# Karthik-Ragunath/RAD-NeRF

Measured on AMD Instinct MI355X. Metric: rendered frames/sec @512x512, higher is better.
Workload: dtype f32; 1 GPU; config[1]: inference 512x512, L=16 hash grid T=2^19 F=2 (xyz; ambient/torso grids tiled T=2^16 as shipped), max 16 steps/ray, 25 FPS pose stream, torso pass on; grid=hash19, engine=fused, frames_per_gpu=2122, table_dtype=f32, audio_batch=8, frames_in_flight=1, loop_launch=split, parallelism=frame-parallel x1

## Files before the change

include/radnerf_fused.h:

```cpp
#ifndef RADNERF_FUSED_H
#define RADNERF_FUSED_H

#include "radnerf_hip.h"

#ifdef __cplusplus
extern "C" {
#endif

typedef struct {
    const void *embeddings;
    const int32_t *offsets;
    uint32_t D, L, H;
    float S;
    uint32_t gridtype;
    int dtype;
} rn_grid_t;

typedef struct {
    const float *amb_w0, *amb_w1, *amb_w2;
    const float *sig_w0, *sig_w1, *sig_w2;
    const float *col_w0, *col_w1;
    uint32_t audio_dim, has_eye, ind_dim;
} rn_nerf_weights_t;

// ... 24 lines not shown
    float min_near;
    const uint8_t *bitfield;
    float bound, dt_gamma;
    uint32_t max_steps, cascade, grid_size;
    float T_thresh;
    float *nears, *fars;
    float *weights_sum, *depth, *image;
    int32_t *rays_alive_a, *rays_alive_b;
    float *rays_t;
    float *xyzs, *dirs, *deltas;
    float *sigmas, *rgbs;
    int32_t *state;
    uint32_t *block_counts;
    int32_t *live_slots;
    uint32_t order_w;
} rn_head_t;

int rn_head_begin(const rn_head_t *h, rn_stream_t stream);
int rn_head_iterate(const rn_head_t *h, const rn_grid_t *grid_xyz, const rn_grid_t *grid_amb, const float *packed,
                    const float *bias, uint32_t first_iter, uint32_t n_iters, int mlp_dtype, rn_stream_t stream);
#define RN_LOOP_FIRST_MARCHED 1u
#define RN_LOOP_CLOSE_FRAME 2u
#define RN_LOOP_COOP 4u
int rn_head_iterate_ex(const rn_head_t *h, const rn_grid_t *grid_xyz, const rn_grid_t *grid_amb, const float *packed,
                       const float *bias, uint32_t first_iter, uint32_t n_iters, int mlp_dtype, uint32_t flags,
                       rn_stream_t stream);
int rn_frame_begin(const rn_head_t *h, const float *pose, float fx, float fy, float cx, float cy, uint32_t W,
                   rn_stream_t stream);
int rn_head_reschedule(const rn_head_t *h, uint32_t iter_done, uint32_t schedule_N, const int32_t *alive_total,
                       rn_stream_t stream);
// ... 24 lines not shown
                         float thresh, const float *poses6, const float *ind_code, float torso_shrink,
                         const rn_torso_weights_t *w, const float *packed, const rn_grid_t *grid_torso, const float *bg_in,
                         float *bg_out, float *torso_alpha, float *image, const float *weights_sum, float *depth,
                         const float *nears, const float *fars, uint8_t *image_u8, rn_stream_t stream);

int rn_torso_mask(const float *bg_coords, uint32_t N, const float *density_grid_torso, uint32_t grid_size, float thresh,
                  uint8_t *mask, rn_stream_t stream);

int rn_blend_frame(float *image, const float *weights_sum, const float *bg, float *depth, const float *nears,
                   const float *fars, uint32_t N, uint8_t *image_u8, rn_stream_t stream);

size_t rn_occupancy_workspace(uint32_t C, uint32_t H);
int rn_occupancy_points(uint32_t C, uint32_t H, float bound, const float *noise, uint32_t seed, float *xyzs, rn_stream_t stream);
int rn_occupancy_update(const float *sigmas, float density_scale, float *density_grid, uint32_t C, uint32_t H, float decay,
                        float density_thresh, uint8_t *bitfield, float *stats, void *workspace, rn_stream_t stream);
int rn_mark_untrained_grid(const float *poses, uint32_t n_poses, uint32_t pose_stride, double fx, double fy, double cx, double cy,
                           uint32_t C, uint32_t H, float bound, float *density_grid, rn_stream_t stream);
int rn_torso_grid_points(uint32_t H, const float *noise, uint32_t seed, float *xys, rn_stream_t stream);
int rn_torso_grid_update(const float *alphas, float *density_grid_torso, uint32_t H, float decay, float *stats, rn_stream_t stream);
uint32_t rn_hash_u01_bits(uint32_t seed, uint32_t idx);

typedef struct {
    const float *conv_w[4], *conv_b[4];
    const float *fc_w[2], *fc_b[2];
    const float *att_conv_w[5], *att_conv_b[5];
    const float *att_fc_w, *att_fc_b;
    uint32_t dim_in, dim_aud, has_att;
} rn_audio_weights_t;
#define RN_AUDIO_SEQ 8
#define RN_AUDIO_WIN 16
// ... 66 lines not shown
```

rad-nerf_amd/csrc/rn_dda_dev.h:

```cpp
#pragma once

#include "rn_common.h"

namespace rn {

constexpr float kSqrt3 = 1.7320508075688772f;


__device__ __forceinline__ int mip_from_pos(float x, float y, float z, float max_cascade) {
    const float mx = fmaxf(fabsf(x), fmaxf(fabsf(y), fabsf(z)));
    int e;
    frexpf(mx, &e);
    return (int)fminf(max_cascade - 1, fmaxf(0.0f, (float)e));
}
__device__ __forceinline__ int mip_from_dt(float dt, float H, float max_cascade) {
    const float mx = (float)((double)(dt * H) * 0.5);
    int e;
    frexpf(mx, &e);
    return (int)fminf(max_cascade - 1, fmaxf(0.0f, (float)e));
}

struct Dda {
    float ox, oy, oz, dx, dy, dz, rdx, rdy, rdz;
    float rH, H3, bound, dt_gamma, dt_min, dt_max, far, Cf, Hf;
// ... 103 lines not shown

    __device__ __forceinline__ void emit(float t, float *xyz, float *dir, float *delta) const {
        EmitSamples{xyz, dir, delta}(*this, 0u, t, clampf(ox + t * dx, -bound, bound), clampf(oy + t * dy, -bound, bound),
                                     clampf(oz + t * dz, -bound, bound), clampf(t * dt_gamma, dt_min, dt_max));
    }

    __device__ __forceinline__ float start(float t, float u) const { return t + clampf(t * dt_gamma, dt_min, dt_max) * u; }

    __device__ __forceinline__ uint32_t march_slot(float t, uint32_t n_step, uint32_t base, float *xyzs, float *dirs, float *deltas) const {
        const uint32_t emitted = walk(t, n_step, EmitSamples{xyzs + (size_t)base * 3, dirs + (size_t)base * 3, deltas + (size_t)base * 2});
        for (uint32_t k = emitted; k < n_step; k++) { deltas[((size_t)base + k) * 2] = 0.0f; deltas[((size_t)base + k) * 2 + 1] = 0.0f; }
        return emitted;
    }
};

}
```

rad-nerf_amd/csrc/rn_head_loop.hip:

```cpp
#include "rn_fused_dev.h"
#include "rn_ray_dev.h"

namespace rn {

constexpr int kLoopBlock = 256;

__device__ __forceinline__ uint32_t policy_n_step(uint32_t N, uint32_t n_alive) {
    uint32_t n_step = n_alive ? N / n_alive : 1u;
    n_step = n_step > 8u ? 8u : n_step;
    return n_step < 1u ? 1u : n_step;
}

__device__ __forceinline__ void next_state(int32_t *st, uint32_t N, uint32_t n_alive, uint32_t step, uint32_t max_steps) {
    const uint32_t n_step = policy_n_step(N, n_alive);
    const bool active = step < max_steps && n_alive > 0;
    st[0] = (int32_t)n_alive;
    st[1] = (int32_t)step;
    st[2] = (int32_t)n_step;
    st[3] = active ? (int32_t)(n_alive * n_step) : 0;
    st[4] = active ? 1 : 0;
    st[5] = 0;
}

__device__ __forceinline__ uint32_t list_live_slots(uint32_t emitted, uint32_t base, int32_t *live_count,
// ... 22 lines not shown
        state[6] = 0;
        for (int i = 8; i < 16; i++) state[i] = 0;
        state[RN_HEAD_ST_HIST] = (int32_t)N;
    }
    if (n >= N) return;
    float near, far;
    begin_ray(n, rays_o + (size_t)n * 3, rays_d + (size_t)n * 3, aabb, min_near, nears, fars, rays_t, weights_sum, depth, image, near, far);
    rays_alive[n] = (int32_t)alive_order(n, order_w);
}

__global__ void __launch_bounds__(kLoopBlock)
k_head_march(const int32_t *__restrict__ st, const int32_t *__restrict__ rays_alive, const float *__restrict__ rays_t,
             const float *__restrict__ rays_o, const float *__restrict__ rays_d, float bound, float dt_gamma,
             uint32_t max_steps, uint32_t C, uint32_t H, const uint8_t *__restrict__ grid,
             const float *__restrict__ fars, float *__restrict__ xyzs, float *__restrict__ dirs, float *__restrict__ deltas, int32_t *__restrict__ stats,
             uint32_t *__restrict__ block_live, int32_t *__restrict__ live_count, int32_t *__restrict__ live_slots) {
    if (!st[4]) return;
    const uint32_t n_alive = (uint32_t)st[0], n_step = (uint32_t)st[2];
    const uint32_t n = blockIdx.x * kLoopBlock + threadIdx.x;
    uint32_t emitted = 0;
    const uint32_t base = n * n_step;
    if (n < n_alive) {
        const int index = rays_alive[n];
        Dda s;
        s.init(rays_o + (size_t)index * 3, rays_d + (size_t)index * 3, bound, dt_gamma, max_steps, C, H, grid, fars[index]);
        emitted = s.march_slot(rays_t[index], n_step, base, xyzs, dirs, deltas);
    }
    __shared__ uint32_t sh[kLoopBlock / kWave + 1];
    const uint32_t total = list_live_slots(emitted, base, live_count, live_slots, sh);
    if (threadIdx.x == 0) block_live[blockIdx.x] = total;
    if (n == 0) { atomicAdd(&stats[RN_HEAD_ST_ITERS], 1); atomicAdd(&stats[RN_HEAD_ST_SLOTS], (int32_t)(n_alive * n_step)); }
}

struct RaySource {
    const float *pose;
    float fx, fy, cx, cy;
    uint32_t W;
};

__global__ void __launch_bounds__(kLoopBlock)
k_frame_begin(RaySource rs, float *__restrict__ rays_o, float *__restrict__ rays_d, const float *__restrict__ aabb, uint32_t N,
              float min_near, uint32_t max_steps, float bound, float dt_gamma, uint32_t C, uint32_t H,
              const uint8_t *__restrict__ grid, float *__restrict__ nears, float *__restrict__ fars, float *__restrict__ weights_sum,
              float *__restrict__ depth, float *__restrict__ image, int32_t *__restrict__ rays_alive, float *__restrict__ rays_t,
              int32_t *__restrict__ state, uint32_t order_w, float *__restrict__ xyzs, float *__restrict__ dirs,
              float *__restrict__ deltas, uint32_t *__restrict__ block_live, int32_t *__restrict__ live_slots) {
    const uint32_t n = blockIdx.x * kLoopBlock + threadIdx.x;
    if (n == 0) {
        next_state(state, N, N, 0, max_steps);
        for (int i = 8; i < 16; i++) state[i] = 0;
        state[RN_HEAD_ST_HIST] = (int32_t)N;
        atomicAdd(&state[RN_HEAD_ST_ITERS], 1);
        atomicAdd(&state[RN_HEAD_ST_SLOTS], (int32_t)N);
    }
    uint32_t emitted = 0;
    if (n < N) {
        const uint32_t ray = alive_order(n, order_w);
        float o[3], d[3];
        if (rs.pose) {
            pinhole_ray(ray, rs.W, rs.fx, rs.fy, rs.cx, rs.cy, rs.pose, o, d);
#pragma unroll
            for (int k = 0; k < 3; k++) { rays_d[(size_t)ray * 3 + k] = d[k]; rays_o[(size_t)ray * 3 + k] = o[k]; }
        } else {
#pragma unroll
            for (int k = 0; k < 3; k++) { o[k] = rays_o[(size_t)ray * 3 + k]; d[k] = rays_d[(size_t)ray * 3 + k]; }
        }
        float near, far;
        begin_ray(ray, o, d, aabb, min_near, nears, fars, rays_t, weights_sum, depth, image, near, far);
        rays_alive[n] = (int32_t)ray;
        Dda s;
        s.init(o, d, bound, dt_gamma, max_steps, C, H, grid, far);
        emitted = s.march_slot(near, 1u, n, xyzs, dirs, deltas);
    }
    __shared__ uint32_t sh[kLoopBlock / kWave + 1];
    const uint32_t total = list_live_slots(emitted, n, state + 6, live_slots, sh);
    if (threadIdx.x == 0) block_live[blockIdx.x] = total;
}

constexpr uint32_t kTagShift = 10;
constexpr uint32_t kTagMask = (1u << 22) - 1u;
constexpr uint32_t kBarrierPolls = 1u << 20;

template <bool COOP>
__device__ __forceinline__ void composite_chunk(uint32_t c, uint32_t n_alive, uint32_t n_step, float T_thresh,
                                                int32_t *__restrict__ rays_alive, float *__restrict__ rays_t,
                                                const float *__restrict__ sigmas, const float *__restrict__ rgbs,
// ... 30 lines not shown
    if (blockIdx.x == 0 && threadIdx.x == 0) st_next[6] = 0;
    const uint32_t n_alive = (uint32_t)st[0], n_step = (uint32_t)st[2];
    if (blockIdx.x * kLoopBlock >= n_alive) return;
    composite_chunk<false>(blockIdx.x, n_alive, n_step, T_thresh, rays_alive, rays_t, sigmas, rgbs, deltas, weights_sum, depth, image,
                           block_counts, wave_cnt);
}

struct MarchArgs {
    const float *rays_t, *rays_o, *rays_d, *fars;
    float bound, dt_gamma;
    uint32_t cascade, grid_size;
    const uint8_t *grid;
    float *xyzs, *dirs, *deltas;
    uint32_t *block_live_next;
    int32_t *live_slots;
};

__device__ __forceinline__ void loop_idle(const int32_t *__restrict__ st, int32_t *__restrict__ st_next, int32_t *__restrict__ stats,
                                          uint32_t close_frame, uint32_t iter) {
    if (blockIdx.x == 0 && threadIdx.x < 8) st_next[threadIdx.x] = st[threadIdx.x];
    if (close_frame && blockIdx.x == 0 && threadIdx.x == 0) { stats[6] = 0; stats[8 + 6] = 0; }
    if (blockIdx.x == 0 && threadIdx.x == 0 && iter + 1 < 32) stats[RN_HEAD_ST_HIST + iter + 1] = 0;
}

template <bool MARCH, bool COOP>
__device__ __forceinline__ void compact_chunk(uint32_t c, uint32_t n_blocks, const int32_t *__restrict__ st, int32_t *__restrict__ st_next,
                                              uint32_t N, uint32_t max_steps, const int32_t *__restrict__ rays_in,
                                              int32_t *__restrict__ rays_out, const uint32_t *__restrict__ block_counts,
                                              const uint32_t *__restrict__ block_live, int32_t *__restrict__ stats, const MarchArgs &m,
                                              uint32_t close_frame, uint32_t iter, uint32_t tag = 0) {
// ... 60 lines not shown
        if (close_frame) {
            if (active_next) atomicAdd(&stats[RN_HEAD_ST_UNFINISHED], 1);
            stats[6] = 0; stats[8 + 6] = 0;
        }
        if (MARCH && active_next) {
            st_next[5] = (int32_t)n_blocks;
            atomicAdd(&stats[RN_HEAD_ST_ITERS], 1);
            atomicAdd(&stats[RN_HEAD_ST_SLOTS], (int32_t)(n_next * n_step_next));
        }
    }
    if constexpr (MARCH) {
        if (!active_next) return;
        uint32_t emitted = 0;
        const uint32_t base = slot * n_step_next;
        if (keep) {
            Dda s;
            s.init(m.rays_o + (size_t)v * 3, m.rays_d + (size_t)v * 3, m.bound, m.dt_gamma, max_steps, m.cascade, m.grid_size, m.grid,
                   m.fars[v]);
            emitted = s.march_slot(m.rays_t[v], n_step_next, base, m.xyzs, m.dirs, m.deltas);
        }
        __shared__ uint32_t sh[kLoopBlock / kWave + 1];
        const uint32_t total = list_live_slots(emitted, base, st_next + 6, m.live_slots, sh);
        if (threadIdx.x == 0) m.block_live_next[c] = total;
    }
}

template <bool MARCH>
__global__ void __launch_bounds__(kLoopBlock)
k_head_compact(const int32_t *__restrict__ st, int32_t *__restrict__ st_next, uint32_t N, uint32_t max_steps,
               const int32_t *__restrict__ rays_in, int32_t *__restrict__ rays_out,
               const uint32_t *__restrict__ block_counts, const uint32_t *__restrict__ block_live, int32_t *__restrict__ stats,
               MarchArgs m, uint32_t close_frame, uint32_t iter) {
    if (!st[4]) { loop_idle(st, st_next, stats, close_frame, iter); return; }
// ... 82 lines not shown
               "head_iterate: mlp_dtype must be RN_F32, RN_F16 or RN_F32_SPLIT");
    RN_REQUIRE(packed && bias && ((uintptr_t)packed & 15u) == 0, "head_iterate: packed/bias");
    if (int rc = check_fused_grid(grid_xyz, 3, "head_iterate(xyz grid)")) return rc;
    if (int rc = check_fused_grid(grid_amb, 2, "head_iterate(ambient grid)")) return rc;
    hipStream_t s = as_stream(stream);
    const dim3 rgrid(div_up(h->N, kLoopBlock)), rblock(kLoopBlock);
    const uint32_t nb = div_up(h->N, kLoopBlock) + 1;
    uint32_t *block_live[2] = {h->block_counts + nb, h->block_counts + 2 * nb};
    for (uint32_t it = first_iter; it < first_iter + n_iters; it++) {
        int32_t *st = h->state + (it & 1u) * 8, *st_next = h->state + ((it + 1) & 1u) * 8;
        int32_t *alive = (it & 1u) ? h->rays_alive_b : h->rays_alive_a;
        int32_t *alive_next = (it & 1u) ? h->rays_alive_a : h->rays_alive_b;
        if (it == first_iter && !(flags & RN_LOOP_FIRST_MARCHED))
            hipLaunchKernelGGL(k_head_march, rgrid, rblock, 0, s, st, alive, h->rays_t, h->rays_o, h->rays_d, h->bound,
                               h->dt_gamma, h->max_steps, h->cascade, h->grid_size, h->bitfield, h->fars, h->xyzs, h->dirs,
                               h->deltas, h->state, block_live[it & 1u], st + 6, h->live_slots);
        run_fused(h->xyzs, h->dirs, h->deltas, h->N, h->live_slots ? st + 6 : st + 3, grid_xyz, grid_amb, packed, bias, h->bound,
                  h->sigmas, h->rgbs, nullptr, mlp_dtype, s, h->live_slots);
        const MarchArgs m{h->rays_t, h->rays_o, h->rays_d, h->fars, h->bound, h->dt_gamma, h->cascade, h->grid_size, h->bitfield,
                          h->xyzs, h->dirs, h->deltas, block_live[(it + 1) & 1u], h->live_slots};
        const bool march_next = it + 1 < first_iter + n_iters;
        const uint32_t close = (!march_next && (flags & RN_LOOP_CLOSE_FRAME)) ? 1u : 0u;
        if (flags & RN_LOOP_COOP) {
            const dim3 cgrid(rgrid.x < kStepGrid ? rgrid.x : kStepGrid);
            uint32_t a_N = h->N, a_max = h->max_steps, a_close = march_next ? 0u : close, a_it = it;
            float a_T = h->T_thresh;
            const int32_t *a_st = st;
            int32_t *a_st_next = st_next, *a_alive = alive, *a_alive_next = alive_next, *a_state = h->state;
            float *a_rays_t = h->rays_t, *a_ws = h->weights_sum, *a_depth = h->depth, *a_image = h->image;
            const float *a_sig = h->sigmas, *a_rgb = h->rgbs, *a_deltas = h->deltas;
            uint32_t *a_counts = h->block_counts;
            const uint32_t *a_live = block_live[it & 1u];
            MarchArgs a_m = m;
            void *args[] = {&a_st, &a_st_next, &a_N, &a_max, &a_T, &a_alive, &a_alive_next, &a_rays_t, &a_sig, &a_rgb, &a_deltas, &a_ws,
                            &a_depth, &a_image, &a_counts, &a_live, &a_state, &a_m, &a_close, &a_it};
// ... 21 lines not shown

int rn_head_iterate(const rn_head_t *h, const rn_grid_t *grid_xyz, const rn_grid_t *grid_amb, const float *packed,
                    const float *bias, uint32_t first_iter, uint32_t n_iters, int mlp_dtype, rn_stream_t stream) {
    return rn_head_iterate_ex(h, grid_xyz, grid_amb, packed, bias, first_iter, n_iters, mlp_dtype, 0u, stream);
}

int rn_frame_begin(const rn_head_t *h, const float *pose, float fx, float fy, float cx, float cy, uint32_t W, rn_stream_t stream) {
    if (int rc = check_head(h)) return rc;
    RN_REQUIRE(!pose || (fx != 0.0f && fy != 0.0f && W >= 1 && h->N % W == 0), "frame_begin: bad intrinsics / image width");
    const uint32_t order_w = usable_order_w(h->order_w, h->N);
    const uint32_t nb = div_up(h->N, kLoopBlock) + 1;
    const RaySource rs{pose, fx, fy, cx, cy, W ? W : 1u};
    hipLaunchKernelGGL(k_frame_begin, dim3(div_up(h->N, kLoopBlock)), dim3(kLoopBlock), 0, as_stream(stream), rs,
                       const_cast<float *>(h->rays_o), const_cast<float *>(h->rays_d), h->aabb, h->N, h->min_near, h->max_steps, h->bound,
                       h->dt_gamma, h->cascade, h->grid_size, h->bitfield, h->nears, h->fars, h->weights_sum, h->depth, h->image,
                       h->rays_alive_a, h->rays_t, h->state, order_w, h->xyzs, h->dirs, h->deltas, h->block_counts + nb, h->live_slots);
    return check_launch("frame_begin");
}

int rn_head_check_done(const rn_head_t *h, uint32_t iters_done, rn_stream_t stream) {
    if (int rc = check_head(h)) return rc;
    hipLaunchKernelGGL(k_head_check_done, dim3(1), dim3(64), 0, as_stream(stream), h->state + (iters_done & 1u) * 8,
                       h->state + RN_HEAD_ST_UNFINISHED);
    return check_launch("head_check_done");
}

int rn_head_reschedule(const rn_head_t *h, uint32_t iter_done, uint32_t schedule_N, const int32_t *alive_total,
                       rn_stream_t stream) {
    if (int rc = check_head(h)) return rc;
    RN_REQUIRE(alive_total && schedule_N >= h->N, "head_reschedule: alive_total is null or schedule_N < N");
    hipLaunchKernelGGL(k_head_reschedule, dim3(1), dim3(64), 0, as_stream(stream), h->state + ((iter_done + 1) & 1u) * 8,
// ... 6 lines not shown
```

rad-nerf_amd/csrc/rn_occupancy.hip:

```cpp
#include "rn_common.h"

#include "../../include/radnerf_fused.h"

#include <math.h>

namespace rn {

constexpr int kOccBlock = 256;

struct CascadeConsts {
    float scale[16];
    float half[16];
};

__global__ void __launch_bounds__(kOccBlock)
k_occ_points(uint32_t C, uint32_t H, CascadeConsts cc, const float *__restrict__ noise, uint32_t seed, float *__restrict__ xyzs) {
    const uint32_t H3 = H * H * H;
    const uint32_t i = blockIdx.x * kOccBlock + threadIdx.x;
    if (i >= C * H3) return;
    const uint32_t cas = i / H3, mo = i - cas * H3;
    const uint32_t c[3] = {morton3D_invert(mo), morton3D_invert(mo >> 1), morton3D_invert(mo >> 2)};
    const float hm1 = (float)(H - 1);
#pragma unroll
    for (int d = 0; d < 3; d++) {
// ... 51 lines not shown
    const uint32_t n = blockIdx.x * kOccBlock + threadIdx.x;
    if (n >= N) return;
    const float thresh = stats[1];
    const float4 a = reinterpret_cast<const float4 *>(grid)[(size_t)n * 2];
    const float4 b = reinterpret_cast<const float4 *>(grid)[(size_t)n * 2 + 1];
    uint32_t bits = 0;
    bits |= (a.x > thresh) ? 1u : 0u;
    bits |= (a.y > thresh) ? 2u : 0u;
    bits |= (a.z > thresh) ? 4u : 0u;
    bits |= (a.w > thresh) ? 8u : 0u;
    bits |= (b.x > thresh) ? 16u : 0u;
    bits |= (b.y > thresh) ? 32u : 0u;
    bits |= (b.z > thresh) ? 64u : 0u;
    bits |= (b.w > thresh) ? 128u : 0u;
    bitfield[n] = (uint8_t)bits;
}

constexpr int kPoseChunk = 64;

__global__ void __launch_bounds__(kOccBlock)
k_mark_untrained(const float *__restrict__ poses, uint32_t n_poses, uint32_t pose_stride, float cx_fx, float cy_fy, uint32_t C,
                 uint32_t H, CascadeConsts cc, float *__restrict__ grid) {
    __shared__ float sp[kPoseChunk][12];
    const uint32_t H3 = H * H * H, total = C * H3;
    const uint32_t i = blockIdx.x * kOccBlock + threadIdx.x;
    const bool in_range = i < total;
    const uint32_t cas = in_range ? i / H3 : 0u, mo = i - cas * H3;
    float w[3] = {0.0f, 0.0f, 0.0f};
    float margin = 0.0f;
    if (in_range) {
// ... 98 lines not shown

int rn_occupancy_update(const float *sigmas, float density_scale, float *density_grid, uint32_t C, uint32_t H, float decay,
                        float density_thresh, uint8_t *bitfield, float *stats, void *workspace, rn_stream_t stream) {
    RN_REQUIRE(sigmas && density_grid && bitfield && stats && workspace, "occupancy_update: null pointer");
    RN_REQUIRE(C >= 1 && C <= 16 && H >= 2 && H <= 1024 && (H * H * H) % 8 == 0, "occupancy_update: bad C / H");
    RN_REQUIRE(((uintptr_t)density_grid & 15u) == 0 && ((uintptr_t)workspace & 7u) == 0, "occupancy_update: alignment");
    const uint32_t total = C * H * H * H, blocks = div_up(total, kOccBlock);
    double *partial = static_cast<double *>(workspace);
    hipStream_t s = as_stream(stream);
    hipLaunchKernelGGL(k_occ_update, dim3(blocks), dim3(kOccBlock), 0, s, sigmas, density_scale, density_grid, C, H, decay, partial);
    hipLaunchKernelGGL(k_occ_mean, dim3(1), dim3(kOccBlock), 0, s, partial, blocks, total, density_thresh, stats);
    hipLaunchKernelGGL(k_occ_pack, dim3(div_up(total / 8, kOccBlock)), dim3(kOccBlock), 0, s, density_grid, total / 8, stats, bitfield);
    return check_launch("occupancy_update");
}

int rn_mark_untrained_grid(const float *poses, uint32_t n_poses, uint32_t pose_stride, double fx, double fy, double cx, double cy,
                           uint32_t C, uint32_t H, float bound, float *density_grid, rn_stream_t stream) {
    RN_REQUIRE(poses && density_grid && n_poses >= 1 && pose_stride >= 12, "mark_untrained_grid: bad arguments");
    RN_REQUIRE(C >= 1 && C <= 16 && H >= 2 && H <= 1024, "mark_untrained_grid: bad C / H");
    const uint32_t total = C * H * H * H;
    hipLaunchKernelGGL(k_mark_untrained, dim3(div_up(total, kOccBlock)), dim3(kOccBlock), 0, as_stream(stream), poses, n_poses,
                       pose_stride, (float)(cx / fx), (float)(cy / fy), C, H,
                       cascade_consts(C, H, (double)bound), density_grid);
    return check_launch("mark_untrained_grid");
}

int rn_torso_grid_points(uint32_t H, const float *noise, uint32_t seed, float *xys, rn_stream_t stream) {
    RN_REQUIRE(xys && H >= 2 && H <= 1024, "torso_grid_points: bad arguments");
    const double half = 1.0 / (double)H;
    hipLaunchKernelGGL(k_torso_points, dim3(div_up(H * H, kOccBlock)), dim3(kOccBlock), 0, as_stream(stream), H, (float)(1.0 - half),
// ... 21 lines not shown
```

rad-nerf_amd/radnerf/fused.py:

```python
import ctypes as C

import numpy as np
import os

import torch

import radnerf_hip as hip
from radnerf_hip.abi import (RN_F16, RN_F32, RN_F32_SPLIT, RN_HEAD_ST_HIST, RN_HEAD_ST_ITERS, RN_HEAD_ST_SLOTS, RN_HEAD_ST_STALLED,
                             RN_HEAD_ST_UNFINISHED, RN_HEAD_STATE_INTS, RN_LOOP_CLOSE_FRAME, RN_LOOP_COOP, RN_LOOP_FIRST_MARCHED,
                             GridT, HeadT, NerfWeightsT, TorsoWeightsT)

_lib = hip._lib


def _grid_desc(enc, table):
    g = GridT()
    g.embeddings, g.offsets = table.data_ptr(), enc.offsets.data_ptr()
    g.D, g.L, g.H = enc.input_dim, enc.num_levels, enc.base_resolution
    g.S = float(np.log2(enc.per_level_scale))
    g.gridtype = enc.gridtype_id
    g.dtype = RN_F16 if table.dtype == torch.float16 else RN_F32
    return g


# ... 46 lines not shown

    def __init__(self, model):
        if not supported(model):
            raise RuntimeError("fused engine: unsupported network shape; use engine='ops'")
        self.model = model
        self.dev = model.density_bitfield.device
        n_packed = max(int(_lib.rn_nerf_packed_floats()), int(_lib.rn_nerf_packed_floats_h16()),
                       int(_lib.rn_nerf_packed_floats_split()))
        self.packed = torch.empty(n_packed, dtype=torch.float32, device=self.dev)
        self.mlp_dtype = RN_F32
        self.loop_hint = None
        self.bias = torch.empty(int(_lib.rn_nerf_bias_floats()), dtype=torch.float32, device=self.dev)
        self.tpacked = (torch.empty(int(_lib.rn_torso_packed_floats()), dtype=torch.float32, device=self.dev)
                        if model.torso else None)
        self._versions = None
        self._N = 0
        self._zero_eye = torch.zeros(1, dtype=torch.float32, device=self.dev)

    def _weights(self):
        m = self.model
        ws = head_weights(m)
        if m.torso:
            ws += torso_weights(m)
        return ws

    def refresh(self):
        ws = self._weights()
        tables = [self.model.encoder.embeddings, self.model.encoder_ambient.embeddings]
        if self.model.torso:
            tables.append(self.model.torso_encoder.embeddings)
        mlp = {"f32": RN_F32, "f16": RN_F16, "f32x2": RN_F32_SPLIT}[
            getattr(getattr(self.model, "opt", None), "mlp_dtype", "f32")]
        half = bool(getattr(getattr(self.model, "opt", None), "half_tables", False))
        versions = tuple((w._version, w.data_ptr()) for w in ws + tables) + (mlp, half)
        if versions == self._versions:
            return
        m = self.model
        for w in ws:
            if w.dtype != torch.float32 or not w.is_contiguous():
                raise RuntimeError("fused engine: MLP weights must be contiguous float32")
        self.nw = weights_desc(ws[:8], m.audio_dim, int(m.exp_eye), m.individual_dim)
# ... 4 lines not shown
                  RN_F32_SPLIT: "rn_nerf_pack_weights_split"}[mlp]
        hip.call(packer, C.byref(self.nw), hip.ptr(self.packed), hip.stream())
        if m.torso:
            self.tw = torso_weights_desc(ws[8:14], m.individual_dim_torso)
            hip.call("rn_torso_pack_weights", C.byref(self.tw), hip.ptr(self.tpacked), hip.stream())
        if half:
            encs = [m.encoder, m.encoder_ambient] + ([m.torso_encoder] if m.torso else [])
            self.tables = [hip.aligned(e.half_table()) for e in encs]
        else:
            self.tables = [hip.aligned(t.detach()) for t in tables]
        self.gx = _grid_desc(m.encoder, self.tables[0])
        self.gw = _grid_desc(m.encoder_ambient, self.tables[1])
        self.gt = _grid_desc(m.torso_encoder, self.tables[2]) if m.torso else None
        self._versions = versions

    def scratch(self, N):
        if N == self._N:
            return
        d, f32, i32 = self.dev, torch.float32, torch.int32
        self.nears = torch.empty(N, dtype=f32, device=d)
        self.fars = torch.empty(N, dtype=f32, device=d)
        self.rays_alive = torch.empty(2, N, dtype=i32, device=d)
        self.rays_t = torch.empty(N, dtype=f32, device=d)
        self.samples = torch.empty(N * 8, dtype=f32, device=d)
        self.sigmas = torch.empty(N, dtype=f32, device=d)
        self.rgbs = torch.empty(N, 3, dtype=f32, device=d)
        self.state = torch.zeros(RN_HEAD_STATE_INTS, dtype=i32, device=d)
        self.stats_prev = [0, 0, 0]
        self.block_counts = torch.zeros(3 * ((N + 255) // 256 + 1), dtype=i32, device=d)
        self.live_slots = torch.empty(N, dtype=i32, device=d)
# ... 202 lines not shown
    h = HeadT()
    h.rays_o, h.rays_d, h.N = rays_o.data_ptr(), rays_d.data_ptr(), N
    h.aabb, h.min_near = model.aabb_infer.data_ptr(), float(model.min_near)
    h.bitfield, h.bound, h.dt_gamma = model.density_bitfield.data_ptr(), float(model.bound), float(dt_gamma)
    h.max_steps, h.cascade, h.grid_size, h.T_thresh = int(max_steps), int(model.cascade), int(model.grid_size), float(T_thresh)
    h.nears, h.fars = st.nears.data_ptr(), st.fars.data_ptr()
    h.weights_sum, h.depth, h.image = weights_sum.data_ptr(), depth.data_ptr(), image.data_ptr()
    h.rays_alive_a, h.rays_alive_b = st.rays_alive[0].data_ptr(), st.rays_alive[1].data_ptr()
    h.rays_t = st.rays_t.data_ptr()
    h.xyzs = st.samples.data_ptr()
    h.dirs = st.samples.data_ptr() + N * 3 * 4
    h.deltas = st.samples.data_ptr() + N * 6 * 4
    h.sigmas, h.rgbs = st.sigmas.data_ptr(), st.rgbs.data_ptr()
    h.state, h.block_counts = st.state.data_ptr(), st.block_counts.data_ptr()
    h.live_slots = st.live_slots.data_ptr() if (getattr(model.opt, "live_list", True) and os.environ.get("RN_LIVE_LIST", "1") != "0") else None
    h.order_w = int(getattr(model, "ray_order_width", 0) or 0)

    shard = getattr(model, "shard_schedule", None)
    merged = shard is None and getattr(model.opt, "frame_kernels", "merged") == "merged"
    n_iters = int(max_steps) if st.loop_hint is None else min(int(max_steps), st.loop_hint)
    if merged:
        if ray_source is not None:
            pose, (fx, fy, cx, cy), W = ray_source
            pose = pose.reshape(-1, 4)[:4].contiguous().float()
            hip.call("rn_frame_begin", C.byref(h), hip.ptr(pose), float(fx), float(fy), float(cx), float(cy), int(W), s)
        else:
            hip.call("rn_frame_begin", C.byref(h), None, 0.0, 0.0, 0.0, 0.0, 0, s)
        hip.call("rn_head_iterate_ex", C.byref(h), C.byref(st.gx), C.byref(st.gw), hip.ptr(st.packed), hip.ptr(bias), 0, n_iters,
                 st.mlp_dtype, RN_LOOP_FIRST_MARCHED | RN_LOOP_CLOSE_FRAME | loop_flags(model), s)
    else:
# ... 80 lines not shown
```

rad-nerf_amd/radnerf/occupancy.py:

```python
import random

import torch

import radnerf_hip as hip

_lib = hip._lib


class _Scratch:

    def __init__(self, model):
        dev = model.density_bitfield.device
        n = model.cascade * model.grid_size ** 3
        self.xyzs = torch.empty(n, 3, dtype=torch.float32, device=dev)
        self.sigmas = torch.empty(n, dtype=torch.float32, device=dev)
        self.stats = torch.zeros(2, dtype=torch.float32, device=dev)
        self.ws = torch.zeros(int(_lib.rn_occupancy_workspace(model.cascade, model.grid_size)), dtype=torch.uint8, device=dev)
        if model.torso:
            g2 = model.grid_size ** 2
            self.xys = torch.empty(g2, 2, dtype=torch.float32, device=dev)
            self.alphas = torch.empty(g2, 1, dtype=torch.float32, device=dev)
            self.bg = torch.empty(g2, 3, dtype=torch.float32, device=dev)
            self.stats_torso = torch.zeros(1, dtype=torch.float32, device=dev)

# ... 13 lines not shown
    if noise.numel() != n * dims:
        raise ValueError(f"jitter noise must hold {n} x {dims} numbers")
    return noise, 0


def _density_into(model, xyzs, sigmas, enc_a, eye):
    from . import fused
    if getattr(model.opt, "grid_refresh_engine", "fused") == "fused" and fused.supported(model):
        fused.density_forward(model, xyzs, enc_a, eye, out=sigmas)
        return
    step = 1 << 19
    for lo in range(0, xyzs.shape[0], step):
        sigmas[lo:lo + step] = model.density(xyzs[lo:lo + step], enc_a, eye)["sigma"].reshape(-1).float()


@torch.no_grad()
def refresh_head(model, enc_a, eye, decay=0.95, noise=None):
    sc = _scratch(model)
    Cc, H = int(model.cascade), int(model.grid_size)
    nz, seed = _jitter(noise, Cc * H ** 3, 3, sc.xyzs.device)
    s = hip.stream()
    hip.call("rn_occupancy_points", Cc, H, float(model.bound), hip.ptr(nz), seed, hip.ptr(sc.xyzs), s)
    _density_into(model, sc.xyzs, sc.sigmas, enc_a, eye)
    grid = model.density_grid
    if not grid.is_contiguous():
        raise RuntimeError("density_grid must be contiguous")
    hip.call("rn_occupancy_update", hip.ptr(sc.sigmas), float(model.density_scale), hip.ptr(grid), Cc, H, float(decay),
             float(model.density_thresh), hip.ptr(model.density_bitfield), hip.ptr(sc.stats), hip.ptr(sc.ws), s)
    return sc.stats


@torch.no_grad()
def refresh_torso(model, enc_a, pose6, ind_code, decay=0.95, noise=None):
    from . import fused
    sc = _scratch(model)
    H = int(model.grid_size)
    nz, seed = _jitter(noise, H * H, 2, sc.xys.device)
    s = hip.stream()
    hip.call("rn_torso_grid_points", H, hip.ptr(nz), seed, hip.ptr(sc.xys), s)
    if fused.supported(model):
        fused.torso_forward(model, sc.xys, pose6, ind_code, thresh=-1.0, bg_out=sc.bg, alpha_out=sc.alphas)
    else:
        sc.alphas.copy_(model.forward_torso(sc.xys, pose6, enc_a, ind_code)[0].float())
# ... 24 lines not shown
```

rad-nerf_amd/radnerf_hip/abi.py:

```python
import ctypes as C

_int, _u32, _f32, _f64, _sz, _ptr, _P = C.c_int, C.c_uint32, C.c_float, C.c_double, C.c_size_t, C.c_void_p, C.POINTER

RN_F32, RN_F16 = 0, 1
RN_LAYOUT_LBC, RN_LAYOUT_BLC, RN_LAYOUT_BLC_LEVELMAJOR = 0, 1, 2

RN_F32_SPLIT = 2
RN_HEAD_STATE_INTS = 64
RN_LOOP_FIRST_MARCHED, RN_LOOP_CLOSE_FRAME, RN_LOOP_COOP = 1, 2, 4
RN_HEAD_ST_ACTIVE, RN_HEAD_ST_ITERS, RN_HEAD_ST_LIVE, RN_HEAD_ST_SLOTS = 4, 16, 17, 18
RN_HEAD_ST_UNFINISHED, RN_HEAD_ST_STALLED, RN_HEAD_ST_HIST = 19, 22, 32


class GridT(C.Structure):
    c_name = "rn_grid_t"
    _fields_ = [("embeddings", _ptr), ("offsets", _ptr), ("D", _u32), ("L", _u32), ("H", _u32), ("S", _f32),
                ("gridtype", _u32), ("dtype", _int)]


class NerfWeightsT(C.Structure):
    c_name = "rn_nerf_weights_t"
    _fields_ = [("amb_w0", _ptr), ("amb_w1", _ptr), ("amb_w2", _ptr), ("sig_w0", _ptr), ("sig_w1", _ptr),
                ("sig_w2", _ptr), ("col_w0", _ptr), ("col_w1", _ptr), ("audio_dim", _u32), ("has_eye", _u32),
                ("ind_dim", _u32)]


class HeadT(C.Structure):
    c_name = "rn_head_t"
    _fields_ = [("rays_o", _ptr), ("rays_d", _ptr), ("N", _u32), ("aabb", _ptr), ("min_near", _f32),
                ("bitfield", _ptr), ("bound", _f32), ("dt_gamma", _f32), ("max_steps", _u32), ("cascade", _u32),
                ("grid_size", _u32), ("T_thresh", _f32), ("nears", _ptr), ("fars", _ptr), ("weights_sum", _ptr),
                ("depth", _ptr), ("image", _ptr), ("rays_alive_a", _ptr), ("rays_alive_b", _ptr), ("rays_t", _ptr),
                ("xyzs", _ptr), ("dirs", _ptr), ("deltas", _ptr), ("sigmas", _ptr), ("rgbs", _ptr), ("state", _ptr),
                ("block_counts", _ptr), ("live_slots", _ptr), ("order_w", _u32)]


class TorsoWeightsT(C.Structure):
    c_name = "rn_torso_weights_t"
    _fields_ = [("def_w0", _ptr), ("def_w1", _ptr), ("def_w2", _ptr), ("tor_w0", _ptr), ("tor_w1", _ptr),
                ("tor_w2", _ptr), ("ind_dim", _u32)]


class AudioWeightsT(C.Structure):
    c_name = "rn_audio_weights_t"
    _fields_ = [("conv_w", _ptr * 4), ("conv_b", _ptr * 4), ("fc_w", _ptr * 2), ("fc_b", _ptr * 2),
                ("att_conv_w", _ptr * 5), ("att_conv_b", _ptr * 5), ("att_fc_w", _ptr), ("att_fc_b", _ptr),
                ("dim_in", _u32), ("dim_aud", _u32), ("has_att", _u32)]


# ... 92 lines not shown
    "rn_head_iterate_ex": (_int, [_P(HeadT), _P(GridT), _P(GridT), _ptr, _ptr, _u32, _u32, _int, _u32, _ptr]),
    "rn_frame_begin": (_int, [_P(HeadT), _ptr, _f32, _f32, _f32, _f32, _u32, _ptr]),
    "rn_head_reschedule": (_int, [_P(HeadT), _u32, _u32, _ptr, _ptr]),
    "rn_head_check_done": (_int, [_P(HeadT), _u32, _ptr]),
    "rn_torso_packed_floats": (_sz, []),
    "rn_torso_pack_weights": (_int, [_P(TorsoWeightsT), _ptr, _ptr]),
    "rn_torso_fused": (_int, [_ptr, _u32, _ptr, _u32, _f32, _ptr, _ptr, _f32, _P(TorsoWeightsT), _ptr, _P(GridT), _ptr, _ptr,
                              _ptr, _ptr, _ptr]),
    "rn_torso_blend_frame": (_int, [_ptr, _u32, _ptr, _u32, _f32, _ptr, _ptr, _f32, _P(TorsoWeightsT), _ptr, _P(GridT), _ptr,
                                    _ptr, _ptr, _ptr, _ptr, _ptr, _ptr, _ptr, _ptr, _ptr]),
    "rn_torso_mask": (_int, [_ptr, _u32, _ptr, _u32, _f32, _ptr, _ptr]),
    "rn_blend_frame": (_int, [_ptr, _ptr, _ptr, _ptr, _ptr, _ptr, _u32, _ptr, _ptr]),
    "rn_occupancy_workspace": (_sz, [_u32, _u32]),
    "rn_occupancy_points": (_int, [_u32, _u32, _f32, _ptr, _u32, _ptr, _ptr]),
    "rn_occupancy_update": (_int, [_ptr, _f32, _ptr, _u32, _u32, _f32, _f32, _ptr, _ptr, _ptr, _ptr]),
    "rn_mark_untrained_grid": (_int, [_ptr, _u32, _u32, _f64, _f64, _f64, _f64, _u32, _u32, _f32, _ptr, _ptr]),
    "rn_torso_grid_points": (_int, [_u32, _ptr, _u32, _ptr, _ptr]),
    "rn_torso_grid_update": (_int, [_ptr, _ptr, _u32, _f32, _ptr, _ptr]),
    "rn_hash_u01_bits": (_u32, [_u32, _u32]),
    "rn_audio_encode_windows": (_int, [_P(AudioWeightsT), _ptr, _u32, _ptr, _ptr, _ptr]),
    "rn_audio_encode_windows_backward": (_int, [_P(AudioWeightsT), _ptr, _u32, _ptr, _ptr, _P(AudioGradsT), _ptr, _ptr]),
    "rn_audio_train_acts_floats": (_sz, [_u32, _int]),
    "rn_audio_encode_windows_train": (_int, [_P(AudioWeightsT), _ptr, _u32, _ptr, _ptr, _ptr, _ptr]),
    "rn_audio_encode_windows_backward_acts": (_int, [_P(AudioWeightsT), _ptr, _u32, _ptr, _ptr, _P(AudioGradsT), _ptr, _ptr,
                                                     _ptr]),
    "rn_audio_encode_stream": (_int, [_P(AudioWeightsT), _ptr, _u32, _u32, _u32, _ptr, _ptr, _ptr]),
    "rn_audio_smooth": (_int, [_ptr, _u32, _u32, _f32, _ptr, _int, _ptr]),
    "rn_audio_smooth_seq": (_int, [_ptr, _u32, _u32, _f32, _ptr, _int, _ptr, _ptr]),
    "rn_get_rays": (_int, [_ptr, _f32, _f32, _f32, _f32, _u32, _u32, _ptr, _ptr, _ptr]),
    "rn_get_bg_coords": (_int, [_u32, _u32, _ptr, _ptr]),
# ... 60 lines not shown
```

Baseline: 1275 frames/s.

## Clip ray marching to the occupied bounding box of the density bitfield

Adds a kernel that reduces the occupancy bitfield to an integer bounding box of occupied cells. The march kernels then clip each ray's far distance to that box and, for single-cascade grids, skip the start forward to the box entry. This aims to cut the empty-space DDA steps and the ray iterations spent outside occupied geometry. It adds a small bounds-refresh kernel whenever the bitfield changes, plus a host sync in refresh. There is some risk of edge mismatches near the box boundaries.

Result: no change. 1287 frames/s, median of 6 (+0.9%).

```diff
diff --git a/include/radnerf_fused.h b/include/radnerf_fused.h
--- a/include/radnerf_fused.h
+++ b/include/radnerf_fused.h
@@ -62,6 +62,7 @@
     uint32_t *block_counts;
     int32_t *live_slots;
     uint32_t order_w;
+    const int32_t *occ_bounds;
 } rn_head_t;
 
 int rn_head_begin(const rn_head_t *h, rn_stream_t stream);
@@ -116,6 +117,7 @@
 int rn_occupancy_points(uint32_t C, uint32_t H, float bound, const float *noise, uint32_t seed, float *xyzs, rn_stream_t stream);
 int rn_occupancy_update(const float *sigmas, float density_scale, float *density_grid, uint32_t C, uint32_t H, float decay,
                         float density_thresh, uint8_t *bitfield, float *stats, void *workspace, rn_stream_t stream);
+int rn_occupancy_bounds(const uint8_t *bitfield, uint32_t C, uint32_t H, int32_t *bounds, rn_stream_t stream);
 int rn_mark_untrained_grid(const float *poses, uint32_t n_poses, uint32_t pose_stride, double fx, double fy, double cx, double cy,
                            uint32_t C, uint32_t H, float bound, float *density_grid, rn_stream_t stream);
 int rn_torso_grid_points(uint32_t H, const float *noise, uint32_t seed, float *xys, rn_stream_t stream);
diff --git a/rad-nerf_amd/csrc/rn_dda_dev.h b/rad-nerf_amd/csrc/rn_dda_dev.h
--- a/rad-nerf_amd/csrc/rn_dda_dev.h
+++ b/rad-nerf_amd/csrc/rn_dda_dev.h
@@ -1,6 +1,7 @@
 #pragma once
 
 #include "rn_common.h"
+#include "rn_occ_clip_dev.h"
 
 namespace rn {
 
@@ -141,4 +142,21 @@
     }
 };
 
+struct DdaClip : Dda {
+    float t_in;
+
+    __device__ __forceinline__ void set_clip(const int32_t *__restrict__ bounds) {
+        const float o[3] = {ox, oy, oz}, rd[3] = {rdx, rdy, rdz};
+        occ_clip_set(bounds, Hf, mb1, o, rd, dt_max, one_step_skips, far, t_in);
+    }
+
+    __device__ __forceinline__ uint32_t march_slot(float t, uint32_t n_step, uint32_t base, float *xyzs, float *dirs, float *deltas) const {
+        if (!occ_clip_advance(t, t_in, far, dt_max)) {
+            for (uint32_t k = 0; k < n_step; k++) { deltas[((size_t)base + k) * 2] = 0.0f; deltas[((size_t)base + k) * 2 + 1] = 0.0f; }
+            return 0u;
+        }
+        return Dda::march_slot(t, n_step, base, xyzs, dirs, deltas);
+    }
+};
+
 }
diff --git a/rad-nerf_amd/csrc/rn_head_loop.hip b/rad-nerf_amd/csrc/rn_head_loop.hip
--- a/rad-nerf_amd/csrc/rn_head_loop.hip
+++ b/rad-nerf_amd/csrc/rn_head_loop.hip
@@ -60,7 +60,8 @@
              const float *__restrict__ rays_o, const float *__restrict__ rays_d, float bound, float dt_gamma,
              uint32_t max_steps, uint32_t C, uint32_t H, const uint8_t *__restrict__ grid,
              const float *__restrict__ fars, float *__restrict__ xyzs, float *__restrict__ dirs, float *__restrict__ deltas, int32_t *__restrict__ stats,
-             uint32_t *__restrict__ block_live, int32_t *__restrict__ live_count, int32_t *__restrict__ live_slots) {
+             uint32_t *__restrict__ block_live, int32_t *__restrict__ live_count, int32_t *__restrict__ live_slots,
+             const int32_t *__restrict__ occ_bounds) {
     if (!st[4]) return;
     const uint32_t n_alive = (uint32_t)st[0], n_step = (uint32_t)st[2];
     const uint32_t n = blockIdx.x * kLoopBlock + threadIdx.x;
@@ -68,8 +69,9 @@
     const uint32_t base = n * n_step;
     if (n < n_alive) {
         const int index = rays_alive[n];
-        Dda s;
+        DdaClip s;
         s.init(rays_o + (size_t)index * 3, rays_d + (size_t)index * 3, bound, dt_gamma, max_steps, C, H, grid, fars[index]);
+        s.set_clip(occ_bounds);
         emitted = s.march_slot(rays_t[index], n_step, base, xyzs, dirs, deltas);
     }
     __shared__ uint32_t sh[kLoopBlock / kWave + 1];
@@ -90,7 +92,8 @@
               const uint8_t *__restrict__ grid, float *__restrict__ nears, float *__restrict__ fars, float *__restrict__ weights_sum,
               float *__restrict__ depth, float *__restrict__ image, int32_t *__restrict__ rays_alive, float *__restrict__ rays_t,
               int32_t *__restrict__ state, uint32_t order_w, float *__restrict__ xyzs, float *__restrict__ dirs,
-              float *__restrict__ deltas, uint32_t *__restrict__ block_live, int32_t *__restrict__ live_slots) {
+              float *__restrict__ deltas, uint32_t *__restrict__ block_live, int32_t *__restrict__ live_slots,
+              const int32_t *__restrict__ occ_bounds) {
     const uint32_t n = blockIdx.x * kLoopBlock + threadIdx.x;
     if (n == 0) {
         next_state(state, N, N, 0, max_steps);
@@ -114,8 +117,9 @@
         float near, far;
         begin_ray(ray, o, d, aabb, min_near, nears, fars, rays_t, weights_sum, depth, image, near, far);
         rays_alive[n] = (int32_t)ray;
-        Dda s;
+        DdaClip s;
         s.init(o, d, bound, dt_gamma, max_steps, C, H, grid, far);
+        s.set_clip(occ_bounds);
         emitted = s.march_slot(near, 1u, n, xyzs, dirs, deltas);
     }
     __shared__ uint32_t sh[kLoopBlock / kWave + 1];
@@ -176,6 +180,7 @@
     float *xyzs, *dirs, *deltas;
     uint32_t *block_live_next;
     int32_t *live_slots;
+    const int32_t *occ_bounds;
 };
 
 __device__ __forceinline__ void loop_idle(const int32_t *__restrict__ st, int32_t *__restrict__ st_next, int32_t *__restrict__ stats,
@@ -266,9 +271,10 @@
         uint32_t emitted = 0;
         const uint32_t base = slot * n_step_next;
         if (keep) {
-            Dda s;
+            DdaClip s;
             s.init(m.rays_o + (size_t)v * 3, m.rays_d + (size_t)v * 3, m.bound, m.dt_gamma, max_steps, m.cascade, m.grid_size, m.grid,
                    m.fars[v]);
+            s.set_clip(m.occ_bounds);
             emitted = s.march_slot(m.rays_t[v], n_step_next, base, m.xyzs, m.dirs, m.deltas);
         }
         __shared__ uint32_t sh[kLoopBlock / kWave + 1];
@@ -381,11 +387,11 @@
         if (it == first_iter && !(flags & RN_LOOP_FIRST_MARCHED))
             hipLaunchKernelGGL(k_head_march, rgrid, rblock, 0, s, st, alive, h->rays_t, h->rays_o, h->rays_d, h->bound,
                                h->dt_gamma, h->max_steps, h->cascade, h->grid_size, h->bitfield, h->fars, h->xyzs, h->dirs,
-                               h->deltas, h->state, block_live[it & 1u], st + 6, h->live_slots);
+                               h->deltas, h->state, block_live[it & 1u], st + 6, h->live_slots, h->occ_bounds);
         run_fused(h->xyzs, h->dirs, h->deltas, h->N, h->live_slots ? st + 6 : st + 3, grid_xyz, grid_amb, packed, bias, h->bound,
                   h->sigmas, h->rgbs, nullptr, mlp_dtype, s, h->live_slots);
         const MarchArgs m{h->rays_t, h->rays_o, h->rays_d, h->fars, h->bound, h->dt_gamma, h->cascade, h->grid_size, h->bitfield,
-                          h->xyzs, h->dirs, h->deltas, block_live[(it + 1) & 1u], h->live_slots};
+                          h->xyzs, h->dirs, h->deltas, block_live[(it + 1) & 1u], h->live_slots, h->occ_bounds};
         const bool march_next = it + 1 < first_iter + n_iters;
         const uint32_t close = (!march_next && (flags & RN_LOOP_CLOSE_FRAME)) ? 1u : 0u;
         if (flags & RN_LOOP_COOP) {
@@ -437,7 +443,8 @@
     hipLaunchKernelGGL(k_frame_begin, dim3(div_up(h->N, kLoopBlock)), dim3(kLoopBlock), 0, as_stream(stream), rs,
                        const_cast<float *>(h->rays_o), const_cast<float *>(h->rays_d), h->aabb, h->N, h->min_near, h->max_steps, h->bound,
                        h->dt_gamma, h->cascade, h->grid_size, h->bitfield, h->nears, h->fars, h->weights_sum, h->depth, h->image,
-                       h->rays_alive_a, h->rays_t, h->state, order_w, h->xyzs, h->dirs, h->deltas, h->block_counts + nb, h->live_slots);
+                       h->rays_alive_a, h->rays_t, h->state, order_w, h->xyzs, h->dirs, h->deltas, h->block_counts + nb, h->live_slots,
+                       h->occ_bounds);
     return check_launch("frame_begin");
 }
 
diff --git a/rad-nerf_amd/csrc/rn_occ_clip_dev.h b/rad-nerf_amd/csrc/rn_occ_clip_dev.h
--- /dev/null
+++ b/rad-nerf_amd/csrc/rn_occ_clip_dev.h
@@ -0,0 +1,54 @@
+#pragma once
+
+#include <math.h>
+#include <stdint.h>
+
+#if defined(__HIPCC__)
+#define RN_CLIP_HD __host__ __device__ __forceinline__
+#else
+#define RN_CLIP_HD inline
+#endif
+
+namespace rn {
+
+RN_CLIP_HD bool occ_clip_interval(const int32_t *bounds, float Hf, float mb1, const float o[3], const float rd[3], float dt,
+                                  float &t_in, float &t_out) {
+    if (!bounds || !bounds[6]) return false;
+    if (bounds[0] > bounds[3] || bounds[1] > bounds[4] || bounds[2] > bounds[5]) {
+        t_in = INFINITY;
+        t_out = -INFINITY;
+        return true;
+    }
+    const float cell = 2.0f / Hf;
+    const int32_t top = (int32_t)Hf - 1;
+    float lo_t = -INFINITY, hi_t = INFINITY;
+    bool ok = true;
+    for (int k = 0; k < 3; k++) {
+        const float f0 = bounds[k] <= 0 ? -INFINITY : ((float)(bounds[k] - 1) * cell - 1.0f) * mb1;
+        const float f1 = bounds[3 + k] >= top ? INFINITY : ((float)(bounds[3 + k] + 2) * cell - 1.0f) * mb1;
+        const float a = (f0 - o[k]) * rd[k], b = (f1 - o[k]) * rd[k];
+        ok = ok && a == a && b == b;
+        lo_t = fmaxf(lo_t, fminf(a, b));
+        hi_t = fminf(hi_t, fmaxf(a, b));
+    }
+    t_in = lo_t - dt;
+    t_out = hi_t + dt;
+    return ok;
+}
+
+RN_CLIP_HD void occ_clip_set(const int32_t *bounds, float Hf, float mb1, const float o[3], const float rd[3], float dt,
+                             bool one_step_skips, float &far, float &t_in) {
+    t_in = -INFINITY;
+    float a, b;
+    if (!occ_clip_interval(bounds, Hf, mb1, o, rd, dt, a, b)) return;
+    if (b < far) far = b;
+    if (one_step_skips) t_in = a;
+}
+
+RN_CLIP_HD bool occ_clip_advance(float &t, float t_in, float far, float dt) {
+    if (!(fmaxf(t, t_in) < far)) return false;
+    for (uint32_t guard = 0; t < t_in && guard < (1u << 19); guard++) t += dt;
+    return true;
+}
+
+}
diff --git a/rad-nerf_amd/csrc/rn_occupancy.hip b/rad-nerf_amd/csrc/rn_occupancy.hip
--- a/rad-nerf_amd/csrc/rn_occupancy.hip
+++ b/rad-nerf_amd/csrc/rn_occupancy.hip
@@ -89,6 +89,36 @@
     bits |= (b.z > thresh) ? 64u : 0u;
     bits |= (b.w > thresh) ? 128u : 0u;
     bitfield[n] = (uint8_t)bits;
+}
+
+__global__ void k_occ_bounds_reset(uint32_t H, int32_t valid, int32_t *__restrict__ bounds) {
+    if (threadIdx.x < 8) bounds[threadIdx.x] = threadIdx.x < 3 ? (int32_t)H : threadIdx.x < 6 ? -1 : threadIdx.x == 6 ? valid : 0;
+}
+
+__global__ void __launch_bounds__(kOccBlock)
+k_occ_bounds(const uint8_t *__restrict__ bitfield, uint32_t N, uint32_t H3, int32_t *__restrict__ bounds) {
+    const uint32_t n = blockIdx.x * kOccBlock + threadIdx.x;
+    const uint32_t bits = n < N ? bitfield[n] : 0u;
+    int32_t lo[3] = {INT32_MAX, INT32_MAX, INT32_MAX}, hi[3] = {-1, -1, -1};
+    if (bits) {
+        const uint32_t mo = (n % (H3 / 8u)) * 8u;
+        const uint32_t zero[3] = {0x55u, 0x33u, 0x0Fu};
+#pragma unroll
+        for (int d = 0; d < 3; d++) {
+            const int32_t c = (int32_t)morton3D_invert(mo >> d);
+            lo[d] = c + ((bits & zero[d]) ? 0 : 1);
+            hi[d] = c + ((bits & ~zero[d] & 0xFFu) ? 1 : 0);
+        }
+    }
+    if (!__ballot(bits != 0u)) return;
+#pragma unroll
+    for (int d = 0; d < 3; d++) {
+        for (int off = 32; off > 0; off >>= 1) {
+            lo[d] = min(lo[d], __shfl_down(lo[d], off, 64));
+            hi[d] = max(hi[d], __shfl_down(hi[d], off, 64));
+        }
+        if ((threadIdx.x & 63) == 0) { atomicMin(&bounds[d], lo[d]); atomicMax(&bounds[3 + d], hi[d]); }
+    }
 }
 
 constexpr int kPoseChunk = 64;
@@ -217,6 +247,16 @@
     return check_launch("occupancy_update");
 }
 
+int rn_occupancy_bounds(const uint8_t *bitfield, uint32_t C, uint32_t H, int32_t *bounds, rn_stream_t stream) {
+    RN_REQUIRE(bitfield && bounds, "occupancy_bounds: null pointer");
+    RN_REQUIRE(C >= 1 && C <= 16 && H >= 2 && H <= 1024 && (H * H * H) % 8 == 0, "occupancy_bounds: bad C / H");
+    const uint32_t H3 = H * H * H, N = C * (H3 / 8);
+    hipStream_t s = as_stream(stream);
+    hipLaunchKernelGGL(k_occ_bounds_reset, dim3(1), dim3(64), 0, s, H, (C == 1 && H <= 256) ? 1 : 0, bounds);
+    hipLaunchKernelGGL(k_occ_bounds, dim3(div_up(N, kOccBlock)), dim3(kOccBlock), 0, s, bitfield, N, H3, bounds);
+    return check_launch("occupancy_bounds");
+}
+
 int rn_mark_untrained_grid(const float *poses, uint32_t n_poses, uint32_t pose_stride, double fx, double fy, double cx, double cy,
                            uint32_t C, uint32_t H, float bound, float *density_grid, rn_stream_t stream) {
     RN_REQUIRE(poses && density_grid && n_poses >= 1 && pose_stride >= 12, "mark_untrained_grid: bad arguments");
diff --git a/rad-nerf_amd/radnerf/fused.py b/rad-nerf_amd/radnerf/fused.py
--- a/rad-nerf_amd/radnerf/fused.py
+++ b/rad-nerf_amd/radnerf/fused.py
@@ -84,6 +84,7 @@
         self.tpacked = (torch.empty(int(_lib.rn_torso_packed_floats()), dtype=torch.float32, device=self.dev)
                         if model.torso else None)
         self._versions = None
+        self.occ_bounds = None
         self._N = 0
         self._zero_eye = torch.zeros(1, dtype=torch.float32, device=self.dev)
 
@@ -95,6 +96,7 @@
         return ws
 
     def refresh(self):
+        self.occ_bounds = self._occ_bounds()
         ws = self._weights()
         tables = [self.model.encoder.embeddings, self.model.encoder_ambient.embeddings]
         if self.model.torso:
@@ -129,6 +131,20 @@
         self.gt = _grid_desc(m.torso_encoder, self.tables[2]) if m.torso else None
         self._versions = versions
 
+    def _occ_bounds(self):
+        from . import occupancy
+        m = self.model
+        bf = m.density_bitfield
+        seen = (bf.data_ptr(), bf._version)
+        if seen != getattr(m, "_occ_bounds_seen", None):
+            if torch.cuda.is_current_stream_capturing():
+                return None
+            torch.cuda.synchronize(bf.device)
+            occupancy.update_bounds(m)
+            torch.cuda.current_stream(bf.device).synchronize()
+            object.__setattr__(m, "_occ_bounds_seen", seen)
+        return occupancy.bounds_buffer(m)
+
     def scratch(self, N):
         if N == self._N:
             return
@@ -361,6 +377,7 @@
     h.sigmas, h.rgbs = st.sigmas.data_ptr(), st.rgbs.data_ptr()
     h.state, h.block_counts = st.state.data_ptr(), st.block_counts.data_ptr()
     h.live_slots = st.live_slots.data_ptr() if (getattr(model.opt, "live_list", True) and os.environ.get("RN_LIVE_LIST", "1") != "0") else None
+    h.occ_bounds = st.occ_bounds.data_ptr() if (st.occ_bounds is not None and os.environ.get("RN_OCC_CLIP", "1") != "0") else None
     h.order_w = int(getattr(model, "ray_order_width", 0) or 0)
 
     shard = getattr(model, "shard_schedule", None)
diff --git a/rad-nerf_amd/radnerf/occupancy.py b/rad-nerf_amd/radnerf/occupancy.py
--- a/rad-nerf_amd/radnerf/occupancy.py
+++ b/rad-nerf_amd/radnerf/occupancy.py
@@ -51,6 +51,21 @@
         sigmas[lo:lo + step] = model.density(xyzs[lo:lo + step], enc_a, eye)["sigma"].reshape(-1).float()
 
 
+def bounds_buffer(model):
+    buf = getattr(model, "_occ_bounds", None)
+    if buf is None or buf.device != model.density_bitfield.device:
+        buf = torch.zeros(8, dtype=torch.int32, device=model.density_bitfield.device)
+        object.__setattr__(model, "_occ_bounds", buf)
+    return buf
+
+
+def update_bounds(model):
+    buf = bounds_buffer(model)
+    hip.call("rn_occupancy_bounds", hip.ptr(model.density_bitfield), int(model.cascade), int(model.grid_size), hip.ptr(buf),
+             hip.stream())
+    return buf
+
+
 @torch.no_grad()
 def refresh_head(model, enc_a, eye, decay=0.95, noise=None):
     sc = _scratch(model)
@@ -64,6 +79,7 @@
         raise RuntimeError("density_grid must be contiguous")
     hip.call("rn_occupancy_update", hip.ptr(sc.sigmas), float(model.density_scale), hip.ptr(grid), Cc, H, float(decay),
              float(model.density_thresh), hip.ptr(model.density_bitfield), hip.ptr(sc.stats), hip.ptr(sc.ws), s)
+    update_bounds(model)
     return sc.stats
 
 
diff --git a/rad-nerf_amd/radnerf_hip/abi.py b/rad-nerf_amd/radnerf_hip/abi.py
--- a/rad-nerf_amd/radnerf_hip/abi.py
+++ b/rad-nerf_amd/radnerf_hip/abi.py
@@ -32,7 +32,7 @@
                 ("grid_size", _u32), ("T_thresh", _f32), ("nears", _ptr), ("fars", _ptr), ("weights_sum", _ptr),
                 ("depth", _ptr), ("image", _ptr), ("rays_alive_a", _ptr), ("rays_alive_b", _ptr), ("rays_t", _ptr),
                 ("xyzs", _ptr), ("dirs", _ptr), ("deltas", _ptr), ("sigmas", _ptr), ("rgbs", _ptr), ("state", _ptr),
-                ("block_counts", _ptr), ("live_slots", _ptr), ("order_w", _u32)]
+                ("block_counts", _ptr), ("live_slots", _ptr), ("order_w", _u32), ("occ_bounds", _ptr)]
 
 
 class TorsoWeightsT(C.Structure):
@@ -155,6 +155,7 @@
     "rn_occupancy_workspace": (_sz, [_u32, _u32]),
     "rn_occupancy_points": (_int, [_u32, _u32, _f32, _ptr, _u32, _ptr, _ptr]),
     "rn_occupancy_update": (_int, [_ptr, _f32, _ptr, _u32, _u32, _f32, _f32, _ptr, _ptr, _ptr, _ptr]),
+    "rn_occupancy_bounds": (_int, [_ptr, _u32, _u32, _ptr, _ptr]),
     "rn_mark_untrained_grid": (_int, [_ptr, _u32, _u32, _f64, _f64, _f64, _f64, _u32, _u32, _f32, _ptr, _ptr]),
     "rn_torso_grid_points": (_int, [_u32, _ptr, _u32, _ptr, _ptr]),
     "rn_torso_grid_update": (_int, [_ptr, _ptr, _u32, _f32, _ptr, _ptr]),
```
